# yhlleo/DWC-GAN

Hardware: AMD Instinct MI355X
Metric: CelebA 128x128 training images/sec (higher is better)
Workload: dtype f32; 1 GPU; BASELINE configs[1]: CelebA-shaped 128x128, per-GPU batch 16, fp32, full iteration (dis_update + gen_update + EMA + LR step), vgg_w=0, stride-1 3x3 / 5x5 and stride-2 4x4 layers (forward, data and weight gradient) as fp32-accurate TWO-plane f16 split products on the f16 MFMA (hi + lo 2^-11 per operand, per-tensor power-of-two scales, 3 products per multiply-add, matrix-core partial sums flushed to; image_size=128, per_gpu_batch=16, global_batch=16, parallelism=dp1

## Files before the change

### dwc-gan_amd/csrc/lstm.hip

```cpp
#include "dwc_common.h"

namespace {

__device__ __forceinline__ float sigmoidf_(float x) { return 1.f / (1.f + expf(-x)); }

template <int MT, int NB>
__device__ __forceinline__ void mfma_rows(const float* __restrict__ a_base, int row0, int a_rows, int a_pitch,
                                          const float* const (&b_rows)[NB], bool b_valid, int K, int q0, int q1,
                                          f32x4 (&acc)[NB][MT]) {
    constexpr int CH = (MT * NB <= 2) ? 8 : ((MT + NB <= 6) ? 5 : 3);
    const int lane = threadIdx.x & 63, r = lane & 15, j = lane >> 4;
    const float* a_row[MT];
    bool a_ok[MT];
#pragma unroll
    for (int m = 0; m < MT; ++m) {
        const int row = row0 + m * 16 + r;
        a_ok[m] = row < a_rows;
        a_row[m] = a_base + (size_t)min(row, a_rows - 1) * a_pitch;
    }
    for (int qc = q0; qc < q1; qc += CH) {
        f32x4 av[CH][MT], bv[CH][NB];
#pragma unroll
        for (int u = 0; u < CH; ++u) {
            const int kc = min(16 * (qc + u) + 4 * j, K - 4);
// ... 478 lines not shown
                if (!mine[k]) continue;
                const int p = threadIdx.x + 256 * k, b = b0 + (p >> 4), u = u0 + (p & 15);
                float* dg = dgates + (dTB + (size_t)t * B + b) * K + u;
                dg[0] = nan; dg[H] = nan; dg[2 * H] = nan; dg[3 * H] = nan;
            }
    }
}

template <typename K>
int lstm_resident_capacity(K kernel, unsigned dyn_lds, int variant) {
    static int cache[16][16];
    int dev = 0;
    if (hipGetDevice(&dev) != hipSuccess) return 0;
    int* slot = (dev >= 0 && dev < 16 && variant >= 0 && variant < 16) ? &cache[dev][variant] : nullptr;
    if (slot && *slot > 0) return *slot;
    int cus = 0, occ = 0;
    if (hipDeviceGetAttribute(&cus, hipDeviceAttributeMultiprocessorCount, dev) != hipSuccess) return 0;
    if (hipOccupancyMaxActiveBlocksPerMultiprocessor(&occ, kernel, 256, dyn_lds) != hipSuccess) return 0;
    const int cap = cus * occ;
    if (slot) *slot = cap;
    return cap;
}

}

extern "C" {

int dwc_lstm_fwd(const float* xproj, const float* w_hh, const int* lens, float* out, float* c, float* gates, int T, int B, int H,
                 int dirs, void* stream) {
    if (T <= 0 || B <= 0 || H <= 0 || (H & 3) || dirs < 1 || dirs > 2) return DWC_EINVAL;
    const int mt = min(4, (B + 15) / 16);
    const dim3 grid((H + 15) / 16, dirs, (B + 16 * mt - 1) / (16 * mt));
    hipStream_t st = (hipStream_t)stream;
    for (int s = 0; s < T; ++s) {
        switch (mt) {
            case 1: hipLaunchKernelGGL(lstm_step_fwd<1>, grid, dim3(256), 0, st, xproj, w_hh, lens, out, c, gates, T, B, H, s); break;
            case 2: hipLaunchKernelGGL(lstm_step_fwd<2>, grid, dim3(256), 0, st, xproj, w_hh, lens, out, c, gates, T, B, H, s); break;
            case 3: hipLaunchKernelGGL(lstm_step_fwd<3>, grid, dim3(256), 0, st, xproj, w_hh, lens, out, c, gates, T, B, H, s); break;
            default: hipLaunchKernelGGL(lstm_step_fwd<4>, grid, dim3(256), 0, st, xproj, w_hh, lens, out, c, gates, T, B, H, s); break;
        }
    }
    DWC_LAUNCH_CHECK();
    return DWC_OK;
}

size_t dwc_lstm_seq_ws_bytes(int B, int dirs) { return ((size_t)(16 + dirs * ((B + 63) / 16 + 1)) * sizeof(unsigned) + 64 + 15) / 16 * 16; }

int dwc_lstm_seq_fwd(const float* xproj, const float* w_hh, const int* lens, float* out, float* c, float* gates, int T, int B, int H,
                     int dirs, void* ws, size_t ws_bytes, unsigned* status, int max_workgroups, void* stream) {
// ... 94 lines not shown
```

### dwc-gan_amd/hipdwc/_lib.py

```python
import ctypes
import os

_HERE = os.path.dirname(os.path.abspath(__file__))
LIB_PATH = os.environ.get("DWC_HIP_LIB") or os.path.join(os.path.dirname(_HERE), "lib", "libdwcgan_hip.so")

c_fp = ctypes.c_void_p
c_int = ctypes.c_int
c_sz = ctypes.c_size_t
c_f = ctypes.c_float
c_u = ctypes.c_uint


class AdvSpec(ctypes.Structure):
    _fields_ = [("target", c_f * 4), ("w_src", c_f * 4), ("w_cls", c_f * 4)]


SIGNATURES = {
    "dwc_version": (c_int, []),
    "dwc_x3_gemm_mode": (c_int, [c_int]),
    "dwc_weight_prepared_elems": (c_sz, [c_int] * 8),
    "dwc_weight_prepare_fwd": (c_int, [c_fp, c_fp, c_int, c_int, c_int, c_int, c_int, c_int, c_fp]),
    "dwc_weight_prepare_dgrad": (c_int, [c_fp, c_fp, c_int, c_int, c_int, c_int, c_int, c_int, c_int, c_fp]),
    "dwc_conv2d_fwd_ws_bytes": (c_sz, [c_int] * 9),
    "dwc_conv2d_fwd": (c_int, [c_fp, c_fp, c_fp, c_fp] + [c_int] * 10 + [c_fp, c_sz, c_fp]),
# ... 54 lines not shown
    "dwc_bf16_conv2d_fwd_ex": (c_int, [c_fp, c_fp, c_fp, c_fp] + [c_int] * 12 + [c_fp]),
    "dwc_bf16_conv2d_bwd_data_ws_bytes": (c_sz, [c_int] * 9),
    "dwc_bf16_conv2d_bwd_data": (c_int, [c_fp, c_fp, c_fp] + [c_int] * 9 + [c_fp, c_sz, c_fp]),
    "dwc_bf16_conv2d_bwd_data_fold": (c_int, [c_fp, c_fp, c_fp, c_fp] + [c_int] * 9 + [c_fp, c_sz, c_fp]),
    "dwc_bf16_reflect_pad_adjoint": (c_int, [c_fp, c_fp, c_int, c_int, c_int, c_int, c_int, c_fp]),
    "dwc_bf16_reflect_pad_adjoint_band": (c_int, [c_fp, c_fp, c_int, c_int, c_int, c_int, c_int, c_fp]),
    "dwc_bf16_conv2d_bwd_data_same_ws_bytes": (c_sz, [c_int] * 8),
    "dwc_bf16_conv2d_bwd_data_same": (c_int, [c_fp] * 4 + [c_int] * 8 + [c_fp, c_sz, c_fp]),
    "dwc_bf16_conv2d_bwd_data_ring": (c_int, [c_fp] * 4 + [c_int] * 8 + [c_fp, c_sz, c_fp]),
    "dwc_bf16_conv2d_same_halo_ok": (c_int, [c_int] * 6),
    "dwc_bf16_conv2d_same_halo": (c_int, [c_fp] * 4 + [c_int] * 8 + [c_fp]),
    "dwc_bf16_conv2d_same_halo_add": (c_int, [c_fp] * 5 + [c_int] * 8 + [c_fp]),
    "dwc_bf16_conv2d_bwd_data_same_fused_ok": (c_int, [c_int] * 6),
    "dwc_bf16_conv2d_bwd_data_same_fused": (c_int, [c_fp] * 4 + [c_int] * 6 + [c_fp]),
    "dwc_weight_refresh_multi": (c_int, [c_fp, c_fp, c_fp, c_int, c_int, c_u, c_fp]),
    "dwc_bf16_conv2d_fwd_zeropad": (c_int, [c_fp, c_fp, c_fp, c_fp] + [c_int] * 10 + [c_fp, c_sz, c_fp]),
    "dwc_bf16_conv2d_bwd_data_zeropad_ws_bytes": (c_sz, [c_int] * 8),
    "dwc_bf16_conv2d_bwd_data_zeropad": (c_int, [c_fp, c_fp, c_fp] + [c_int] * 8 + [c_fp, c_sz, c_fp]),
    "dwc_bf16_maxpool2_fwd": (c_int, [c_fp, c_fp, c_int, c_int, c_int, c_int, c_fp]),
    "dwc_bf16_maxpool2_bwd": (c_int, [c_fp, c_fp, c_fp, c_int, c_int, c_int, c_int, c_fp]),
    "dwc_lstm_seq_ws_bytes": (c_sz, [c_int, c_int]),
    "dwc_lstm_seq_fwd": (c_int, [c_fp] * 6 + [c_int] * 4 + [c_fp, c_sz, c_fp, c_int, c_fp]),
    "dwc_lstm_seq_bwd": (c_int, [c_fp] * 7 + [c_int] * 4 + [c_fp, c_sz, c_fp, c_int, c_fp]),
    "dwc_adv_tail_fwd": (c_int, [c_fp, c_fp, c_fp, c_fp, c_int, c_int, c_int, c_int, AdvSpec, c_fp]),
    "dwc_adv_tail_bwd": (c_int, [c_fp, c_fp, c_fp, c_fp, c_fp, c_fp, c_int, c_int, c_int, c_int, AdvSpec, c_fp]),
    "dwc_bf16_conv2d_s2_halo_ok": (c_int, [c_int] * 5),
    "dwc_bf16_conv2d_s2_halo": (c_int, [c_fp] * 4 + [c_int] * 6 + [c_fp]),
    "dwc_x3_conv2d_same_ok": (c_int, [c_int] * 6),
    "dwc_x3_weight_prepared_elems": (c_sz, [c_int] * 3),
    "dwc_x3_weight_prepare": (c_int, [c_fp, c_fp] + [c_int] * 5 + [c_fp]),
    "dwc_x3_conv2d_same": (c_int, [c_fp] * 4 + [c_int] * 9 + [c_fp]),
    "dwc_x3_conv2d_same_add": (c_int, [c_fp] * 5 + [c_int] * 9 + [c_fp]),
    "dwc_x3_conv2d_narrow_ok": (c_int, [c_int] * 8),
    "dwc_x3_conv2d_narrow_weight_elems": (c_sz, [c_int] * 2),
    "dwc_x3_conv2d_narrow": (c_int, [c_fp] * 4 + [c_int] * 12 + [c_fp]),
    "dwc_reflect_pad_adjoint_pitch": (c_int, [c_fp, c_fp] + [c_int] * 6 + [c_fp]),
    "dwc_x3_gather_split": (c_int, [c_fp, c_fp, c_fp, c_int, c_fp]),
    "dwc_x3_conv2d_stem_ok": (c_int, [c_int] * 7),
    "dwc_x3_conv2d_stem_weight_elems": (c_sz, []),
    "dwc_x3_conv2d_stem": (c_int, [c_fp] * 4 + [c_int] * 9 + [c_fp]),
    "dwc_x3_conv2d_stem_crop": (c_int, [c_fp] * 5 + [c_int] * 10 + [c_fp]),
    "dwc_x3_conv2d_stem_amax": (c_int, [c_fp] * 5 + [c_u] + [c_int] * 9 + [c_fp]),
    "dwc_reflect_pad_adjoint_band": (c_int, [c_fp, c_fp, c_int, c_int, c_int, c_int, c_int, c_fp]),
    "dwc_x3_conv2d_ksplit_ws_bytes": (c_sz, [c_int] * 7),
    "dwc_x3_conv2d_ksplit_ticket_words": (c_int, []),
    "dwc_x3_conv2d_same_add_ws": (c_int, [c_fp] * 5 + [c_int] * 9 + [c_fp, c_sz, c_fp, c_fp]),
# ... 50 lines not shown
    "dwc_bf16_upsample2x_bwd": (c_int, [c_fp, c_fp, c_int, c_int, c_int, c_int, c_fp]),
    "dwc_bf16_avgpool2_fwd": (c_int, [c_fp, c_fp, c_int, c_int, c_int, c_int, c_fp]),
    "dwc_bf16_avgpool2_bwd": (c_int, [c_fp, c_fp, c_int, c_int, c_int, c_int, c_fp]),
    "dwc_pack_nchw_to_nhwc8_bf16": (c_int, [c_fp, c_fp, c_int, c_int, c_int, c_int, c_fp]),
    "dwc_unpack_nhwc8_bf16_to_nchw": (c_int, [c_fp, c_fp, c_int, c_int, c_int, c_int, c_fp]),
    "dwc_bf16_blend_fwd": (c_int, [c_fp, c_fp, c_fp, c_int, c_fp]),
    "dwc_bf16_blend_bwd": (c_int, [c_fp, c_fp, c_fp, c_fp, c_int, c_fp]),
    "dwc_bf16_l1_mean_fwd": (c_int, [c_fp, c_fp, c_fp, c_sz, c_int, c_fp, c_sz, c_fp]),
    "dwc_bf16_l1_mean_bwd": (c_int, [c_fp, c_fp, c_fp, c_fp, c_fp, c_sz, c_int, c_fp]),
    "dwc_sn_layer_saved_floats": (c_sz, [c_int] * 3),
    "dwc_sn_power_blocks": (c_int, [c_int, c_int, c_fp, c_fp]),
    "dwc_sn_power_iteration": (c_int, [c_fp, c_int, c_int, c_int, c_fp, c_int, c_fp]),
    "dwc_sn_epilogue_bwd_ws_bytes": (c_sz, [c_int] * 4),
    "dwc_sn_epilogue_fwd": (c_int, [c_fp] * 4 + [c_int] * 4 + [c_fp, c_u, c_fp]),
    "dwc_bf16_sn_epilogue_fwd": (c_int, [c_fp] * 4 + [c_int] * 4 + [c_fp]),
    "dwc_sn_epilogue_bwd": (c_int, [c_fp] * 7 + [c_int] * 4 + [c_fp, c_sz, c_fp, c_u, c_fp]),
    "dwc_bf16_sn_epilogue_bwd": (c_int, [c_fp] * 7 + [c_int] * 4 + [c_fp, c_sz, c_fp]),
    "dwc_sn_weight_grad": (c_int, [c_fp, c_int, c_fp, c_int, c_fp, c_fp, c_fp] + [c_int] * 4 + [c_fp]),
    "dwc_grad_penalty_fwd": (c_int, [c_fp] * 4 + [c_int] * 5 + [c_fp]),
    "dwc_grad_penalty_scale": (c_int, [c_fp] * 4 + [c_int] * 4 + [c_fp]),
    "dwc_src_head_seed": (c_int, [c_fp] * 3 + [c_int] * 3 + [c_fp]),
}

ABI_VERSION = 9
EINVAL = -1
_ERRORS = {-1: "DWC_EINVAL (unsupported shape/argument)", -2: "DWC_EWORKSPACE (scratch too small)",
           -3: "DWC_ELAUNCH (kernel launch failed)"}

_lib = None


class HipKernelError(RuntimeError):
    pass


def load():
    global _lib
    if _lib is not None:
        return _lib
    if not os.path.exists(LIB_PATH):
        raise ImportError(
            "libdwcgan_hip.so not found at %s — build it with `make -C dwc-gan_amd/csrc` "
            "(or python -c 'import __graft_entry__ as g; g.build()'). There is no CPU fallback." % LIB_PATH)
    import torch
    lib = ctypes.CDLL(LIB_PATH)
    for name, (res, args) in SIGNATURES.items():
        fn = getattr(lib, name)
# ... 14 lines not shown
```

### dwc-gan_amd/hipdwc/ops.py

```python
import os
import weakref

import numpy as np
import torch

from . import _lib

ACT = {"none": 0, None: 0, "relu": 1, "lrelu": 2, "tanh": 3, "sigmoid": 4, "heads": 5, "heads8": 6}

PRECISION = "fp32"
BF16 = torch.bfloat16

_REMOVED_SWITCHES = ("DWC_WINOGRAD", "DWC_TXT_STREAM", "DWC_NORM_FUSED_FINAL", "DWC_GEMM_TILE", "DWC_STRIP_BM", "DWC_X3_DUO", "DWC_X3_BN",
                     "DWC_X3_BN32", "DWC_X3_WIDE", "DWC_X3_STAGGER", "DWC_HALO_STAGGER", "DWC_X3_WDUO", "DWC_HALO16", "DWC_HALO_DUO",
                     "DWC_HALO_BN128", "DWC_BF16_TILE", "DWC_BF16_STAGES3", "DWC_NARROW_ROWS16")
_set = [k for k in _REMOVED_SWITCHES if k in os.environ]
if _set:
    import warnings
    warnings.warn("hipdwc: %s no longer select%s anything (removed in round 5, DESIGN.md 10.3) and %s ignored" % (
        ", ".join(_set), "s" if len(_set) == 1 else "", "is" if len(_set) == 1 else "are"), stacklevel=2)
del _set


def set_precision(name):
# ... 450 lines not shown
    _lib.check(lib.dwc_weight_refresh_multi(table[0].data_ptr(), table[1].data_ptr(), table[2].data_ptr(), table[3], table[4],
                                            _REFRESH_EPOCH, _stream()), "weight_refresh_multi")
    for p, ent, key, val, stamp in todo:
        ent[key] = (stamp, val[1], val[2])
    REFRESH_STATS["launches"] += 1
    REFRESH_STATS["layouts"] += len(todo)
    return len(todo)


X3 = int(os.environ.get("DWC_X3", "2"))
HALO = int(os.environ.get("DWC_BF16_HALO", "1"))
WGRAD_HALO = int(os.environ.get("DWC_BF16_WGRAD_HALO", "1"))
STEM = int(os.environ.get("DWC_BF16_STEM", "1"))
NARROW = int(os.environ.get("DWC_BF16_NARROW", "1"))
NARROW_X3 = int(os.environ.get("DWC_X3_NARROW", "1"))
SMALLK_X3 = int(os.environ.get("DWC_X3_SMALLK", "1"))
LSTM_SEQ = int(os.environ.get("DWC_LSTM_SEQ", "1"))
DGRAD_FOLD = int(os.environ.get("DWC_DGRAD_FOLD", "1"))
X3_S2 = int(os.environ.get("DWC_X3_S2", "1"))
S2HALO = int(os.environ.get("DWC_BF16_S2_HALO", "1"))
S2DGRAD = int(os.environ.get("DWC_S2_DGRAD_HALO", "1"))
X3_WGRAD_HALO3 = int(os.environ.get("DWC_X3_WGRAD_HALO3", "1"))
PINNED_STAGE = int(os.environ.get("DWC_PINNED_STAGE", "1"))
ZERO_GRAD_BY_FLAG = int(os.environ.get("DWC_ZERO_GRAD_FLAG", "1"))
RING_FUSED = int(os.environ.get("DWC_RING_FUSED", "1"))
PENALTY_HIP = int(os.environ.get("DWC_PENALTY_HIP", "0"))
S2DGRAD_MIN_WGS = 192


X3_PLANES = int(os.environ.get("DWC_X3_PLANES", "2"))
AMAX_SLOTS = 1 << 16
_AMAX = {}


def amax_slot(dev):
    key = dev.index if dev.index is not None else torch.cuda.current_device()
    pool = _AMAX.get(key)
    if pool is None:
        pool = [torch.zeros(AMAX_SLOTS, dtype=torch.int64, device=dev), 0]
        _AMAX[key] = pool
    i = pool[1]
    pool[1] = i + 1
    return pool[0].data_ptr() + 8 * (i % AMAX_SLOTS), i // AMAX_SLOTS + 1


def amax_live(t, c=False):
# ... 972 lines not shown
            ws = workspace(lib.dwc_lstm_seq_ws_bytes(B, 2), dev)
            rc = lib.dwc_lstm_seq_bwd(_p(d_out), _p(d_c), w_hh_t.data_ptr(), lens.data_ptr(), c.data_ptr(), gates.data_ptr(),
                                      dgates.data_ptr(), T, B, H, 2, ws.data_ptr(), ws.numel(), _lstm_status(dev)[0].data_ptr(),
                                      LSTM_SEQ_MAX_WORKGROUPS, _stream())
            if rc not in (0, _lib.EINVAL):
                _lib.check(rc, "lstm_seq_bwd")
        if rc != 0:
            _lib.check(lib.dwc_lstm_bwd(_p(d_out), _p(d_c), w_hh_t.data_ptr(), lens.data_ptr(), c.data_ptr(), gates.data_ptr(),
                                        dgates.data_ptr(), carry.data_ptr(), T, B, H, 2, _stream()), "lstm_bwd")
        dG = dgates.view(2, T * B, 4 * H)
        dGt = dG.transpose(1, 2)
        hip = ctx.hip_gemm
        dw_ih = None
        if ctx.needs_input_grad[2]:
            if hip:
                dw_ih = torch.empty((2, 4 * H, I), dtype=torch.float32, device=dev)
                for d in range(2):
                    _gemm_tn(dG[d], X, out=dw_ih[d])
            else:
                dw_ih = torch.matmul(dGt, X)
        db = dG.sum(1) if (ctx.needs_input_grad[4] or ctx.needs_input_grad[5]) else None
        dw_hh = None
        if ctx.needs_input_grad[3]:
            hprev = torch.zeros((2, T, B, H), dtype=torch.float32, device=dev)
            hprev[0, 1:] = out[0, :-1]
            hprev[1, :-1] = out[1, 1:]
            hp = hprev.view(2, T * B, H)
            if hip:
                dw_hh = torch.empty((2, 4 * H, H), dtype=torch.float32, device=dev)
                for d in range(2):
                    _gemm_tn(dG[d], hp[d], out=dw_hh[d])
            else:
                dw_hh = torch.bmm(dGt, hp)
        dx = None
        if ctx.needs_input_grad[0]:
            if hip:
                dx = (_gemm_nn(dG[0], w_ih[0], ctx.owners[0]) + _gemm_nn(dG[1], w_ih[1], ctx.owners[1])).view(T, B, I)
            else:
                dx = torch.bmm(dG, w_ih).sum(0).view(T, B, I)
        return dx, None, dw_ih, dw_hh, db, db, None


def lstm_bidir(x, lens, w_ih, w_hh, b_ih, b_hh, owners=None):
    return _LSTMBidir.apply(x.contiguous(), lens, w_ih, w_hh, b_ih, b_hh, owners)


class _InstNorm(torch.autograd.Function):
    @staticmethod
    def forward(ctx, x, gamma, beta, residual, relu, eps, token=None):
        _require_device(x)
        ctx.token = token if residual is not None else None
        lib = _lib.load()
        x = cl(x)
        B, C, H, W = x.shape
        dev = x.device
        if gamma is not None:
            gamma, beta = gamma.float().contiguous(), beta.float().contiguous()
        if residual is not None:
            residual = cl(residual.to(x.dtype))
        y = empty_cl(B, C, H, W, dev, x.dtype)
        mean = torch.empty(B * C, dtype=torch.float32, device=dev)
        rstd = torch.empty(B * C, dtype=torch.float32, device=dev)
        ws = workspace(lib.dwc_instnorm_ws_bytes(B, H * W, C), dev)
        ya, yep = out_amax(y)
        if ya is not None:
            _lib.check(lib.dwc_instnorm_fwd_amax(x.data_ptr(), _p(gamma), _p(beta), _p(residual), y.data_ptr(), mean.data_ptr(),
                                                 rstd.data_ptr(), B, H * W, C, eps, int(relu), ws.data_ptr(), ws.numel(),
# ... 360 lines not shown
```

### dwc-gan_amd/networks/networks_v2.py

```python
import numpy as np
import torch
from torch import nn

from hipdwc import host, ops
from .networks import ContentEncoder, MLP, Conv2dBlock, ResBlocks, AdaptiveInstanceNorm2d, Decoder


class HeadList(list):
    flat = None

    @classmethod
    def of(cls, flat, k):
        out = cls(flat.reshape(flat.shape[0], k, -1).unbind(1))
        out.flat = flat
        return out

    def rows(self, a, b):
        return HeadList.of(self.flat[a:b], len(self))


def flat_heads(heads):
    if torch.is_tensor(heads):
        return heads
    flat = getattr(heads, "flat", None)
# ... 81 lines not shown
            self.embed_tokens.weight.requires_grad = False
        self.lstm = nn.LSTM(input_size=embed_dim + self.style_dim, hidden_size=hidden_size, num_layers=num_layers,
                            dropout=dropout_out if num_layers > 1 else 0.0, bidirectional=bidirectional)
        feat = hidden_size * num_layers * (4 if bidirectional else 2)
        self.fcs, self.fcvars = nn.ModuleList(), nn.ModuleList()
        for _ in range(num_class):
            self.fcs.append(nn.Linear(feat, c_dim))
            self.fcvars.append(nn.Linear(feat, c_dim))

    def forward(self, style_ord, src_tokens, src_lengths):
        noise = host.noise()
        tokens = src_tokens.transpose(1, 0)
        seq_len, bsz = tokens.shape
        lens_host = src_lengths.detach().to("cpu")
        lens_sorted, order_host = torch.sort(lens_host, descending=True)
        if tokens.is_cuda and ops.PINNED_STAGE:
            stage = torch.empty(4, bsz, dtype=torch.int64).pin_memory()
            stage[0], stage[1], stage[2], stage[3] = order_host, torch.sort(order_host)[1], lens_sorted, lens_sorted - 1
            on_dev = stage.to(tokens.device, non_blocking=True)
            order, unsort, lens_dev, last = on_dev[0], on_dev[1], on_dev[2].to(torch.int32), on_dev[3]
        else:
            order, unsort = order_host.to(tokens.device), torch.sort(order_host)[1].to(tokens.device)
            lens_dev, last = lens_sorted.to(torch.int32).to(tokens.device), (lens_sorted - 1).to(tokens.device)
        emb = self.embed_tokens(tokens.index_select(1, order))
        emb = noise.dropout(emb, self.dropout_in, self.training)
        sty = _Permute.apply(style_ord, 0, order, unsort)
        lens_list = lens_sorted.tolist()
        t_max = int(lens_list[0])
        data = torch.cat([emb, sty.expand(seq_len, -1, -1)], -1)[:t_max]
        cols = torch.arange(bsz, device=tokens.device)
        suffixes = ("", "_reverse") if self.bidirectional else ("",)
        if not self.bidirectional:
            raise NotImplementedError("the HIP text encoder is bidirectional (the reference's only configuration)")
        hs, cs = [], []
        for l in range(self.num_layers):
            par = {n: ops.cat_params([getattr(self.lstm, "%s_l%d%s" % (n, l, suf)) for suf in suffixes], stack=True)
                   for n in ("weight_ih", "weight_hh", "bias_ih", "bias_hh")}
            out, cell = ops.lstm_bidir(data, lens_dev, par["weight_ih"], par["weight_hh"], par["bias_ih"], par["bias_hh"],
                                       owners=tuple(getattr(self.lstm, "weight_ih_l%d%s" % (l, suf)) for suf in suffixes))
            hs += [out[0][last, cols], out[1][0]]
            cs += [cell[0][last, cols], cell[1][0]]
            data = torch.cat([out[0], out[1]], -1)
            if l + 1 < self.num_layers and self.training and self.dropout_out > 0:
                if getattr(noise, "align_stream", False):
                    mask = noise.dropout_mask((int(sum(lens_list)), data.shape[2]), self.dropout_out, data.device)
                    data = data * mask.index_select(0, _packed_index(lens_list, t_max, bsz, data.device)).view(t_max, bsz, -1)
                else:
                    data = noise.dropout(data, self.dropout_out, True)
        h_n, c_n = torch.stack(hs), torch.stack(cs)
        if self.training and self.dropout_out > 0 and noise.align_stream:
            noise.dropout(data, self.dropout_out, True)
        h_n = h_n.view(self.num_layers, 2, bsz, -1).transpose(1, 2).reshape(self.num_layers, bsz, -1)
        c_n = c_n.view(self.num_layers, 2, bsz, -1).transpose(1, 2).reshape(self.num_layers, bsz, -1)
        h_n, c_n = _Permute.apply(h_n, 1, unsort, order), _Permute.apply(c_n, 1, unsort, order)
        feat = torch.cat([h_n, c_n], dim=1).view(bsz, -1)
        w = ops.cat_params([m.weight for m in self.fcs] + [m.weight for m in self.fcvars])
        b = ops.cat_params([m.bias for m in self.fcs] + [m.bias for m in self.fcvars])
        if feat.is_cuda and ops.LSTM_GEMM and ops.gemm_ok(feat.shape[1], w.shape[0]):
            out = ops.linear_any(feat, w, b, owner=tuple(m.weight for m in self.fcs) + tuple(m.weight for m in self.fcvars))
        else:
            out = torch.nn.functional.linear(feat, w, b)
        k, c = self.num_class, self.style_dim // self.num_class
        return HeadList.of(out[:, :k * c], k), HeadList.of(out[:, k * c:2 * k * c], k)


class AdaINGen_v2(nn.Module):

    def __init__(self, input_dim, vocab, params, pretrained_embed=None):
        super().__init__()
        p = params
        style_dim = p["c_dim"] * p["num_cls"]
        self.enc_style = StyleEncoder(p["style_downsample"], input_dim, p["dim"], norm="none", activ=p["activ"],
                                      pad_type=p["pad_type"], c_dim=p["c_dim"], num_class=p["num_cls"],
                                      use_map=p["use_map"])
        self.enc_content = ContentEncoder(p["content_downsample"], p["n_res"], input_dim, p["dim"], "in", p["activ"],
                                          pad_type=p["pad_type"])
        self.dec = Decoder(p["content_downsample"], p["n_res"], self.enc_content.output_dim, input_dim,
                           res_norm="adain", activ=p["activ"], pad_type=p["pad_type"],
# ... 50 lines not shown
```

### include/dwcgan_hip.h

```cpp
#ifndef DWCGAN_HIP_H
#define DWCGAN_HIP_H

#include <stddef.h>
#include <stdint.h>

#ifdef __cplusplus
extern "C" {
#endif

#define DWC_OK 0
#define DWC_EINVAL (-1)
#define DWC_EWORKSPACE (-2)
#define DWC_ELAUNCH (-3)

#define DWC_ACT_NONE 0
#define DWC_ACT_RELU 1
#define DWC_ACT_LRELU 2
#define DWC_ACT_TANH 3
#define DWC_ACT_SIGMOID 4
#define DWC_ACT_HEADS 5
#define DWC_ACT_HEADS8 6

#define DWC_ABI_VERSION 9
int dwc_version(void);
int dwc_x3_gemm_mode(int mode);

size_t dwc_weight_prepared_elems(int Cout, int Cin, int KH, int KW, int stride, int cout_pad, int cin_pad,
                                 int for_dgrad);
int dwc_weight_prepare_fwd(const float* w_oihw, float* w_prepared, int Cout, int Cin, int KH, int KW,
                           int cout_pad, int cin_pad, void* stream);
int dwc_weight_prepare_dgrad(const float* w_oihw, float* w_prepared, int Cout, int Cin, int KH, int KW,
                             int stride, int cout_pad, int cin_pad, void* stream);

size_t dwc_conv2d_fwd_ws_bytes(int B, int H, int W, int Cin, int Cout, int KH, int KW, int stride, int pad);
int dwc_conv2d_fwd(const float* x, const float* w_prepared, const float* bias, float* y,
                   int B, int H, int W, int Cin, int Cout, int KH, int KW, int stride, int pad,
                   int act, void* ws, size_t ws_bytes, void* stream);
size_t dwc_conv2d_bwd_data_ws_bytes(int B, int H, int W, int Cin, int Cout, int KH, int KW, int stride, int pad);
int dwc_conv2d_bwd_data(const float* dy, const float* w_dgrad, float* dxp,
                        int B, int H, int W, int Cin, int Cout, int KH, int KW, int stride, int pad,
                        void* ws, size_t ws_bytes, void* stream);
int dwc_reflect_pad_adjoint(const float* dxp, float* dx, int B, int H, int W, int C, int pad,
                            void* stream);
int dwc_conv2d_bwd_data_fold(const float* dy, const float* w_dgrad, float* dxp, float* dx, int B, int H, int W, int Cin, int Cout, int KH,
                             int KW, int stride, int pad, void* ws, size_t ws_bytes, void* stream);
size_t dwc_conv2d_bwd_data_same_ws_bytes(int B, int H, int W, int Cin, int Cout, int KH, int KW, int pad);
// ... 69 lines not shown
                  void* stream);

int dwc_gmm_kl_sp_fwd(const float* mu, const float* lv, const float* centre, int centre_stride, int B, int K, int D, float sigma,
                      float* out_scalar, void* stream);
int dwc_gmm_kl_sp_bwd(const float* mu, const float* lv, const float* centre, int centre_stride, int B, int K, int D, float sigma,
                      const float* dout_scalar, float* dmu, float* dlv, void* stream);

size_t dwc_l1_ws_bytes(size_t n);
int dwc_l1_mean_fwd(const float* a, const float* b, float* out_scalar, size_t n, int skip4, void* ws,
                    size_t ws_bytes, void* stream);
int dwc_l1_mean_bwd(const float* a, const float* b, const float* dout_scalar, float* da, float* db,
                    size_t n, int skip4, void* stream);

int dwc_lstm_fwd(const float* xproj, const float* w_hh, const int* lens, float* out, float* c, float* gates,
                 int T, int B, int H, int dirs, void* stream);
size_t dwc_lstm_seq_ws_bytes(int B, int dirs);
int dwc_lstm_seq_fwd(const float* xproj, const float* w_hh, const int* lens, float* out, float* c, float* gates, int T, int B, int H,
                     int dirs, void* ws, size_t ws_bytes, unsigned* status, int max_workgroups, void* stream);
int dwc_lstm_seq_bwd(const float* d_out, const float* d_c, const float* w_hh_t, const int* lens, const float* c, const float* gates,
                     float* dgates, int T, int B, int H, int dirs, void* ws, size_t ws_bytes, unsigned* status, int max_workgroups,
                     void* stream);
int dwc_lstm_bwd(const float* d_out, const float* d_c, const float* w_hh_t, const int* lens, const float* c,
                 const float* gates, float* dgates, float* dc_carry, int T, int B, int H, int dirs, void* stream);

int dwc_adam_step(float* p, const float* g, float* m, float* v, size_t n, float lr, float beta1,
                  float beta2, float eps, float weight_decay, int step, void* stream);
int dwc_ema_lerp(const float* p, float* ema, size_t n, float beta, void* stream);

#define DWC_OPT_CHUNK 8192
typedef struct {
    float* p;
    const float* g;
    float* m;
    float* v;
    unsigned long long n;
    float step_size;
    float bc2_sqrt;
} dwc_adam_tensor;
typedef struct {
    const float* p;
    float* ema;
    unsigned long long n;
} dwc_ema_tensor;
int dwc_adam_multi(const dwc_adam_tensor* tensors_dev, const int* chunk_tensor_dev,
                   const unsigned* chunk_start_dev, int n_chunks, double beta1, double beta2, double eps,
                   double weight_decay, void* stream);
// ... 235 lines not shown
```

Before: 398.3 images/s.

## Fuse text-encoder input assembly and final-state gather into HIP kernels

Adds HIP kernels that build the LSTM input in one pass: embedding lookup, token reordering, dropout mask and style concatenation. A second kernel gathers the final hidden and cell states and unsorts them, with matching backward kernels. The recurrent weight gradient now uses offset views of the outputs instead of materialising a zero-padded shifted copy. All of this replaces many small torch ops (index_select, cat, stack, permute) with fewer launches, at the cost of new custom autograd paths with fallbacks.

After: 401.1 images/s, median of 6. Within noise of the previous version (+0.7%).

```diff
diff --git a/dwc-gan_amd/csrc/lstm.hip b/dwc-gan_amd/csrc/lstm.hip
--- a/dwc-gan_amd/csrc/lstm.hip
+++ b/dwc-gan_amd/csrc/lstm.hip
@@ -524,9 +524,177 @@
     return cap;
 }
 
+
+constexpr int TXT_MAX_LAYERS = DWC_TXT_MAX_LAYERS;
+struct TxtStates { const float* out[TXT_MAX_LAYERS]; const float* c[TXT_MAX_LAYERS]; };
+struct TxtStateGrads { float* d_out[TXT_MAX_LAYERS]; float* d_c[TXT_MAX_LAYERS]; const float* addend[TXT_MAX_LAYERS]; };
+
+__global__ __launch_bounds__(256) void txt_input_fwd(const float* __restrict__ table, const long long* __restrict__ tokens,
+                                                     const long long* __restrict__ order, const float* __restrict__ mask,
+                                                     const float* __restrict__ style, float* __restrict__ data,
+                                                     long long* __restrict__ tok_t, int seq_len, int t_max, int B, int E, int S, int V) {
+    const int W = E + S;
+    const size_t n = (size_t)t_max * B * W, stride = (size_t)gridDim.x * 256;
+    const size_t i0 = (size_t)blockIdx.x * 256 + threadIdx.x;
+    for (size_t i = i0; i < n; i += stride) {
+        const int k = (int)(i % W);
+        const size_t row = i / W;
+        const int j = (int)(row % B), t = (int)(row / B);
+        const long long src = order[j];
+        float v = __builtin_nanf("");
+        if (src >= 0 && src < B) {
+            if (k < E) {
+                const long long tok = tokens[(size_t)src * seq_len + t];
+                if (tok >= 0 && tok < V) {
+                    v = table[(size_t)tok * E + k];
+                    if (mask) v = __fmul_rn(v, mask[row * E + k]);
+                }
+            } else {
+                v = style[(size_t)src * S + (k - E)];
+            }
+        }
+        data[i] = v;
+    }
+    if (tok_t) {
+        const size_t m = (size_t)seq_len * B;
+        for (size_t i = i0; i < m; i += stride) tok_t[i] = tokens[(i % B) * seq_len + i / B];
+    }
+}
+
+__global__ __launch_bounds__(256) void txt_input_bwd(const float* __restrict__ d_data, const long long* __restrict__ unsort,
+                                                     const float* __restrict__ mask, float* __restrict__ d_style,
+                                                     float* __restrict__ d_rows, int seq_len, int t_max, int B, int E, int S) {
+    const int W = E + S;
+    const size_t n_rows = d_rows ? (size_t)seq_len * B * E : 0, n_sty = d_style ? (size_t)B * S : 0;
+    const size_t stride = (size_t)gridDim.x * 256;
+    for (size_t i = (size_t)blockIdx.x * 256 + threadIdx.x; i < n_rows + n_sty; i += stride) {
+        if (i < n_rows) {
+            const int k = (int)(i % E);
+            const size_t row = i / E;
+            const int b = (int)(row % B), t = (int)(row / B);
+            const long long j = unsort[b];
+            float v = 0.f;
+            if (j < 0 || j >= B) {
+                v = __builtin_nanf("");
+            } else if (t < t_max) {
+                const size_t r = (size_t)t * B + j;
+                v = d_data[r * W + k];
+                if (mask) v = __fmul_rn(v, mask[r * E + k]);
+            }
+            d_rows[i] = v;
+        } else {
+            const size_t q = i - n_rows;
+            const int s = (int)(q % S), b = (int)(q / S);
+            const long long j = unsort[b];
+            float acc = 0.f;
+            if (j < 0 || j >= B) {
+                acc = __builtin_nanf("");
+            } else {
+                for (int t = 0; t < t_max; ++t) acc += d_data[((size_t)t * B + j) * W + E + s];
+            }
+            d_style[q] = acc;
+        }
+    }
+}
+
+__global__ __launch_bounds__(256) void txt_final_fwd(TxtStates p, const long long* __restrict__ last, const long long* __restrict__ unsort,
+                                                     float* __restrict__ feat, int L, int T, int B, int H) {
+    const size_t n = (size_t)L * 2 * B * 2 * H, stride = (size_t)gridDim.x * 256;
+    for (size_t i = (size_t)blockIdx.x * 256 + threadIdx.x; i < n; i += stride) {
+        const int k = (int)(i % (2 * H));
+        const int r = (int)((i / (2 * H)) % (2 * B)), l = (int)(i / ((size_t)4 * H * B));
+        const int d = k / H, h = k - d * H, b = r < B ? r : r - B;
+        const float* src = r < B ? p.out[l] : p.c[l];
+        const long long j = unsort[b];
+        float v = __builtin_nanf("");
+        if (j >= 0 && j < B) {
+            const long long t = d == 0 ? last[j] : 0;
+            if (t >= 0 && t < T) v = src[(((size_t)d * T + t) * B + j) * H + h];
+        }
+        feat[i] = v;
+    }
+}
+
+__global__ __launch_bounds__(256) void txt_final_bwd(TxtStateGrads p, const float* __restrict__ d_feat, const long long* __restrict__ last,
+                                                     const long long* __restrict__ order, int L, int T, int B, int H) {
+    const size_t per = (size_t)2 * T * B * H, n = (size_t)L * 2 * per, stride = (size_t)gridDim.x * 256;
+    for (size_t i = (size_t)blockIdx.x * 256 + threadIdx.x; i < n; i += stride) {
+        const size_t e = i % per;
+        const int which = (int)((i / per) & 1), l = (int)(i / (2 * per));
+        const int h = (int)(e % H), j = (int)((e / H) % B), t = (int)((e / ((size_t)H * B)) % T), d = (int)(e / ((size_t)H * B * T));
+        float v = 0.f;
+        if (d == 0 ? (long long)t == last[j] : t == 0) {
+            const long long b = order[j];
+            v = (b >= 0 && b < B) ? d_feat[(((size_t)l * 2 + which) * B + b) * 2 * H + d * H + h] : __builtin_nanf("");
+        }
+        if (which == 0) {
+            if (p.addend[l]) v += p.addend[l][((size_t)t * B + j) * 2 * H + d * H + h];
+            p.d_out[l][e] = v;
+        } else {
+            p.d_c[l][e] = v;
+        }
+    }
+}
+
+inline unsigned txt_blocks(size_t n) { return (unsigned)min((n + 255) / 256, (size_t)4096); }
+
 }
 
 extern "C" {
+
+int dwc_txt_input_fwd(const float* table, const long long* tokens, const long long* order, const float* mask, const float* style,
+                      float* data, long long* tok_t, int seq_len, int t_max, int B, int E, int S, int V, void* stream) {
+    if (!table || !tokens || !order || !style || !data) return DWC_EINVAL;
+    if (seq_len <= 0 || t_max <= 0 || t_max > seq_len || B <= 0 || E <= 0 || S <= 0 || V <= 0) return DWC_EINVAL;
+    if ((size_t)seq_len * B * (E + S) >= 0x80000000ull || (size_t)V * E >= 0x80000000ull) return DWC_EINVAL;
+    const size_t n = max((size_t)t_max * B * (E + S), tok_t ? (size_t)seq_len * B : (size_t)0);
+    hipLaunchKernelGGL(txt_input_fwd, dim3(txt_blocks(n)), dim3(256), 0, (hipStream_t)stream, table, tokens, order, mask, style, data,
+                       tok_t, seq_len, t_max, B, E, S, V);
+    DWC_LAUNCH_CHECK();
+    return DWC_OK;
+}
+
+int dwc_txt_input_bwd(const float* d_data, const long long* unsort, const float* mask, float* d_style, float* d_rows, int seq_len,
+                      int t_max, int B, int E, int S, void* stream) {
+    if (!d_data || !unsort || (!d_style && !d_rows)) return DWC_EINVAL;
+    if (seq_len <= 0 || t_max <= 0 || t_max > seq_len || B <= 0 || E <= 0 || S <= 0) return DWC_EINVAL;
+    if ((size_t)seq_len * B * (E + S) >= 0x80000000ull) return DWC_EINVAL;
+    const size_t n = (d_rows ? (size_t)seq_len * B * E : 0) + (d_style ? (size_t)B * S : 0);
+    hipLaunchKernelGGL(txt_input_bwd, dim3(txt_blocks(n)), dim3(256), 0, (hipStream_t)stream, d_data, unsort, mask, d_style, d_rows,
+                       seq_len, t_max, B, E, S);
+    DWC_LAUNCH_CHECK();
+    return DWC_OK;
+}
+
+int dwc_txt_final_fwd(const float* const* outs, const float* const* cs, const long long* last, const long long* unsort, float* feat,
+                      int L, int T, int B, int H, void* stream) {
+    if (!outs || !cs || !last || !unsort || !feat || L <= 0 || L > TXT_MAX_LAYERS || T <= 0 || B <= 0 || H <= 0) return DWC_EINVAL;
+    if ((size_t)2 * T * B * H >= 0x80000000ull || (size_t)L * 4 * B * H >= 0x80000000ull) return DWC_EINVAL;
+    TxtStates p = {};
+    for (int l = 0; l < L; ++l) {
+        if (!outs[l] || !cs[l]) return DWC_EINVAL;
+        p.out[l] = outs[l], p.c[l] = cs[l];
+    }
+    hipLaunchKernelGGL(txt_final_fwd, dim3(txt_blocks((size_t)L * 4 * B * H)), dim3(256), 0, (hipStream_t)stream, p, last, unsort, feat,
+                       L, T, B, H);
+    DWC_LAUNCH_CHECK();
+    return DWC_OK;
+}
+
+int dwc_txt_final_bwd(const float* d_feat, const long long* last, const long long* order, float* const* d_outs, float* const* d_cs,
+                      const float* const* addends, int L, int T, int B, int H, void* stream) {
+    if (!d_feat || !last || !order || !d_outs || !d_cs || L <= 0 || L > TXT_MAX_LAYERS || T <= 0 || B <= 0 || H <= 0) return DWC_EINVAL;
+    if ((size_t)2 * T * B * H >= 0x80000000ull || (size_t)L * 4 * B * H >= 0x80000000ull) return DWC_EINVAL;
+    TxtStateGrads p = {};
+    for (int l = 0; l < L; ++l) {
+        if (!d_outs[l] || !d_cs[l]) return DWC_EINVAL;
+        p.d_out[l] = d_outs[l], p.d_c[l] = d_cs[l], p.addend[l] = addends ? addends[l] : nullptr;
+    }
+    hipLaunchKernelGGL(txt_final_bwd, dim3(txt_blocks((size_t)L * 4 * T * B * H)), dim3(256), 0, (hipStream_t)stream, p, d_feat, last,
+                       order, L, T, B, H);
+    DWC_LAUNCH_CHECK();
+    return DWC_OK;
+}
 
 int dwc_lstm_fwd(const float* xproj, const float* w_hh, const int* lens, float* out, float* c, float* gates, int T, int B, int H,
                  int dirs, void* stream) {
diff --git a/dwc-gan_amd/hipdwc/_lib.py b/dwc-gan_amd/hipdwc/_lib.py
--- a/dwc-gan_amd/hipdwc/_lib.py
+++ b/dwc-gan_amd/hipdwc/_lib.py
@@ -100,6 +100,10 @@
     "dwc_lstm_seq_ws_bytes": (c_sz, [c_int, c_int]),
     "dwc_lstm_seq_fwd": (c_int, [c_fp] * 6 + [c_int] * 4 + [c_fp, c_sz, c_fp, c_int, c_fp]),
     "dwc_lstm_seq_bwd": (c_int, [c_fp] * 7 + [c_int] * 4 + [c_fp, c_sz, c_fp, c_int, c_fp]),
+    "dwc_txt_input_fwd": (c_int, [c_fp] * 7 + [c_int] * 6 + [c_fp]),
+    "dwc_txt_input_bwd": (c_int, [c_fp] * 5 + [c_int] * 5 + [c_fp]),
+    "dwc_txt_final_fwd": (c_int, [c_fp] * 5 + [c_int] * 4 + [c_fp]),
+    "dwc_txt_final_bwd": (c_int, [c_fp] * 6 + [c_int] * 4 + [c_fp]),
     "dwc_adv_tail_fwd": (c_int, [c_fp, c_fp, c_fp, c_fp, c_int, c_int, c_int, c_int, AdvSpec, c_fp]),
     "dwc_adv_tail_bwd": (c_int, [c_fp, c_fp, c_fp, c_fp, c_fp, c_fp, c_int, c_int, c_int, c_int, AdvSpec, c_fp]),
     "dwc_bf16_conv2d_s2_halo_ok": (c_int, [c_int] * 5),
@@ -196,7 +200,7 @@
     "dwc_src_head_seed": (c_int, [c_fp] * 3 + [c_int] * 3 + [c_fp]),
 }
 
-ABI_VERSION = 9
+ABI_VERSION = 10
 EINVAL = -1
 _ERRORS = {-1: "DWC_EINVAL (unsupported shape/argument)", -2: "DWC_EWORKSPACE (scratch too small)",
            -3: "DWC_ELAUNCH (kernel launch failed)"}
diff --git a/dwc-gan_amd/hipdwc/ops.py b/dwc-gan_amd/hipdwc/ops.py
--- a/dwc-gan_amd/hipdwc/ops.py
+++ b/dwc-gan_amd/hipdwc/ops.py
@@ -1,3 +1,4 @@
+import ctypes
 import os
 import weakref
 
@@ -496,6 +497,7 @@
 S2DGRAD = int(os.environ.get("DWC_S2_DGRAD_HALO", "1"))
 X3_WGRAD_HALO3 = int(os.environ.get("DWC_X3_WGRAD_HALO3", "1"))
 PINNED_STAGE = int(os.environ.get("DWC_PINNED_STAGE", "1"))
+TXT_FUSED = int(os.environ.get("DWC_TXT_FUSED", "1"))
 ZERO_GRAD_BY_FLAG = int(os.environ.get("DWC_ZERO_GRAD_FLAG", "1"))
 RING_FUSED = int(os.environ.get("DWC_RING_FUSED", "1"))
 PENALTY_HIP = int(os.environ.get("DWC_PENALTY_HIP", "0"))
@@ -1514,16 +1516,22 @@
         db = dG.sum(1) if (ctx.needs_input_grad[4] or ctx.needs_input_grad[5]) else None
         dw_hh = None
         if ctx.needs_input_grad[3]:
-            hprev = torch.zeros((2, T, B, H), dtype=torch.float32, device=dev)
-            hprev[0, 1:] = out[0, :-1]
-            hprev[1, :-1] = out[1, 1:]
-            hp = hprev.view(2, T * B, H)
-            if hip:
+            if hip and TXT_FUSED and T > 1:
                 dw_hh = torch.empty((2, 4 * H, H), dtype=torch.float32, device=dev)
-                for d in range(2):
-                    _gemm_tn(dG[d], hp[d], out=dw_hh[d])
+                o = out.view(2, T * B, H)
+                _gemm_tn(dG[0, B:], o[0, :(T - 1) * B], out=dw_hh[0])
+                _gemm_tn(dG[1, :(T - 1) * B], o[1, B:], out=dw_hh[1])
             else:
-                dw_hh = torch.bmm(dGt, hp)
+                hprev = torch.zeros((2, T, B, H), dtype=torch.float32, device=dev)
+                hprev[0, 1:] = out[0, :-1]
+                hprev[1, :-1] = out[1, 1:]
+                hp = hprev.view(2, T * B, H)
+                if hip:
+                    dw_hh = torch.empty((2, 4 * H, H), dtype=torch.float32, device=dev)
+                    for d in range(2):
+                        _gemm_tn(dG[d], hp[d], out=dw_hh[d])
+                else:
+                    dw_hh = torch.bmm(dGt, hp)
         dx = None
         if ctx.needs_input_grad[0]:
             if hip:
@@ -1535,6 +1543,105 @@
 
 def lstm_bidir(x, lens, w_ih, w_hh, b_ih, b_hh, owners=None):
     return _LSTMBidir.apply(x.contiguous(), lens, w_ih, w_hh, b_ih, b_hh, owners)
+
+
+class _TxtUnsupported(Exception):
+    """A dwc_txt_* entry point returned DWC_EINVAL: the caller assembles the tensor with torch ops."""
+
+
+def _txt_call(rc, what):
+    if rc == _lib.EINVAL:
+        raise _TxtUnsupported(what)
+    _lib.check(rc, what)
+
+
+def _ptr_array(tensors):
+    return (ctypes.c_void_p * len(tensors))(*[_p(t) for t in tensors])
+
+
+class _TxtInput(torch.autograd.Function):
+
+    @staticmethod
+    def forward(ctx, table, style, tokens, order, unsort, mask, t_max, padding_idx):
+        B, seq_len = tokens.shape
+        (V, E), S = table.shape, style.shape[1]
+        data = torch.empty((t_max, B, E + S), dtype=torch.float32, device=table.device)
+        tok_t = torch.empty((seq_len, B), dtype=torch.int64, device=table.device) if ctx.needs_input_grad[0] else None
+        _txt_call(_lib.load().dwc_txt_input_fwd(table.data_ptr(), tokens.data_ptr(), order.data_ptr(), _p(mask), style.data_ptr(),
+                                                data.data_ptr(), _p(tok_t), seq_len, t_max, B, E, S, V, _stream()), "txt_input_fwd")
+        ctx.save_for_backward(unsort, mask, tok_t)
+        ctx.dims = (seq_len, t_max, B, E, S, V, -1 if padding_idx is None else int(padding_idx))
+        return data
+
+    @staticmethod
+    def backward(ctx, d_data):
+        unsort, mask, tok_t = ctx.saved_tensors
+        seq_len, t_max, B, E, S, V, pad = ctx.dims
+        d_data = d_data.contiguous()
+        dev = d_data.device
+        d_rows = torch.empty((seq_len, B, E), dtype=torch.float32, device=dev) if ctx.needs_input_grad[0] else None
+        d_style = torch.empty((B, S), dtype=torch.float32, device=dev) if ctx.needs_input_grad[1] else None
+        if d_rows is not None or d_style is not None:
+            _lib.check(_lib.load().dwc_txt_input_bwd(d_data.data_ptr(), unsort.data_ptr(), _p(mask), _p(d_style), _p(d_rows), seq_len,
+                                                     t_max, B, E, S, _stream()), "txt_input_bwd")
+        d_table = None if d_rows is None else torch.ops.aten.embedding_dense_backward(d_rows, tok_t, V, pad, False)
+        return d_table, d_style, None, None, None, None, None, None
+
+
+def _txt_plain(*tensors):
+    return all(t is None or (t.is_cuda and t.is_contiguous()) for t in tensors)
+
+
+def txt_input(table, padding_idx, tokens, order, unsort, mask, style, t_max):
+    if not (TXT_FUSED and _txt_plain(table, tokens, order, unsort, mask, style) and tokens.dtype == torch.int64
+            and order.dtype == torch.int64 and unsort.dtype == torch.int64 and table.dtype == torch.float32
+            and style.dtype == torch.float32 and (mask is None or mask.dtype == torch.float32)):
+        return None
+    try:
+        return _TxtInput.apply(table, style, tokens, order, unsort, mask, int(t_max), padding_idx)
+    except _TxtUnsupported:
+        return None
+
+
+class _TxtFinal(torch.autograd.Function):
+
+    @staticmethod
+    def forward(ctx, last, unsort, order, *states):
+        L = len(states) // 2
+        _, T, B, H = states[0].shape
+        feat = torch.empty((B, 4 * L * H), dtype=torch.float32, device=states[0].device)
+        _txt_call(_lib.load().dwc_txt_final_fwd(_ptr_array(states[0::2]), _ptr_array(states[1::2]), last.data_ptr(), unsort.data_ptr(),
+                                                feat.data_ptr(), L, T, B, H, _stream()), "txt_final_fwd")
+        ctx.save_for_backward(last, order)
+        ctx.dims = (L, T, B, H)
+        return feat
+
+    @staticmethod
+    def backward(ctx, d_feat):
+        last, order = ctx.saved_tensors
+        L, T, B, H = ctx.dims
+        grads = txt_final_bwd(d_feat.contiguous(), last, order, L, T, H)
+        return (None, None, None) + tuple(g for pair in zip(*grads) for g in pair)
+
+
+def txt_final_bwd(d_feat, last, order, L, T, H, addends=None):
+    B = d_feat.shape[0]
+    d_outs = [torch.empty((2, T, B, H), dtype=torch.float32, device=d_feat.device) for _ in range(L)]
+    d_cs = [torch.empty((2, T, B, H), dtype=torch.float32, device=d_feat.device) for _ in range(L)]
+    _lib.check(_lib.load().dwc_txt_final_bwd(d_feat.data_ptr(), last.data_ptr(), order.data_ptr(), _ptr_array(d_outs), _ptr_array(d_cs),
+                                             None if addends is None else _ptr_array(addends), L, T, B, H, _stream()), "txt_final_bwd")
+    return d_outs, d_cs
+
+
+def txt_final(last, unsort, order, outs, cells):
+    states = [t for pair in zip(outs, cells) for t in pair]
+    if not (TXT_FUSED and _txt_plain(last, unsort, order, *states) and all(t.dtype == torch.float32 for t in states)
+            and all(t.dtype == torch.int64 for t in (last, unsort, order))):
+        return None
+    try:
+        return _TxtFinal.apply(last, unsort, order, *states)
+    except _TxtUnsupported:
+        return None
 
 
 class _InstNorm(torch.autograd.Function):
diff --git a/dwc-gan_amd/networks/networks_v2.py b/dwc-gan_amd/networks/networks_v2.py
--- a/dwc-gan_amd/networks/networks_v2.py
+++ b/dwc-gan_amd/networks/networks_v2.py
@@ -127,38 +127,52 @@
         else:
             order, unsort = order_host.to(tokens.device), torch.sort(order_host)[1].to(tokens.device)
             lens_dev, last = lens_sorted.to(torch.int32).to(tokens.device), (lens_sorted - 1).to(tokens.device)
-        emb = self.embed_tokens(tokens.index_select(1, order))
-        emb = noise.dropout(emb, self.dropout_in, self.training)
-        sty = _Permute.apply(style_ord, 0, order, unsort)
         lens_list = lens_sorted.tolist()
         t_max = int(lens_list[0])
-        data = torch.cat([emb, sty.expand(seq_len, -1, -1)], -1)[:t_max]
-        cols = torch.arange(bsz, device=tokens.device)
+        fused = tokens.is_cuda and ops.TXT_FUSED
+        data = mask = None
+        if fused:
+            if self.training and self.dropout_in > 0:
+                mask = noise.dropout_mask((seq_len, bsz, self.embed_dim), self.dropout_in, tokens.device)
+            data = ops.txt_input(self.embed_tokens.weight, self.embed_tokens.padding_idx, src_tokens.contiguous(), order, unsort, mask,
+                                 style_ord, t_max)
+        if data is None:
+            emb = self.embed_tokens(tokens.index_select(1, order))
+            emb = emb * mask if mask is not None else noise.dropout(emb, self.dropout_in, self.training)
+            sty = _Permute.apply(style_ord, 0, order, unsort)
+            data = torch.cat([emb, sty.expand(seq_len, -1, -1)], -1)[:t_max]
         suffixes = ("", "_reverse") if self.bidirectional else ("",)
         if not self.bidirectional:
             raise NotImplementedError("the HIP text encoder is bidirectional (the reference's only configuration)")
-        hs, cs = [], []
+        outs, cells = [], []
         for l in range(self.num_layers):
             par = {n: ops.cat_params([getattr(self.lstm, "%s_l%d%s" % (n, l, suf)) for suf in suffixes], stack=True)
                    for n in ("weight_ih", "weight_hh", "bias_ih", "bias_hh")}
             out, cell = ops.lstm_bidir(data, lens_dev, par["weight_ih"], par["weight_hh"], par["bias_ih"], par["bias_hh"],
                                        owners=tuple(getattr(self.lstm, "weight_ih_l%d%s" % (l, suf)) for suf in suffixes))
-            hs += [out[0][last, cols], out[1][0]]
-            cs += [cell[0][last, cols], cell[1][0]]
-            data = torch.cat([out[0], out[1]], -1)
+            outs.append(out)
+            cells.append(cell)
+            if fused and l + 1 == self.num_layers and not noise.align_stream:
+                break
+            data = out.permute(1, 2, 0, 3).reshape(t_max, bsz, -1) if fused else torch.cat([out[0], out[1]], -1)
             if l + 1 < self.num_layers and self.training and self.dropout_out > 0:
                 if getattr(noise, "align_stream", False):
-                    mask = noise.dropout_mask((int(sum(lens_list)), data.shape[2]), self.dropout_out, data.device)
-                    data = data * mask.index_select(0, _packed_index(lens_list, t_max, bsz, data.device)).view(t_max, bsz, -1)
+                    pmask = noise.dropout_mask((int(sum(lens_list)), data.shape[2]), self.dropout_out, data.device)
+                    data = data * pmask.index_select(0, _packed_index(lens_list, t_max, bsz, data.device)).view(t_max, bsz, -1)
                 else:
                     data = noise.dropout(data, self.dropout_out, True)
-        h_n, c_n = torch.stack(hs), torch.stack(cs)
         if self.training and self.dropout_out > 0 and noise.align_stream:
             noise.dropout(data, self.dropout_out, True)
-        h_n = h_n.view(self.num_layers, 2, bsz, -1).transpose(1, 2).reshape(self.num_layers, bsz, -1)
-        c_n = c_n.view(self.num_layers, 2, bsz, -1).transpose(1, 2).reshape(self.num_layers, bsz, -1)
-        h_n, c_n = _Permute.apply(h_n, 1, unsort, order), _Permute.apply(c_n, 1, unsort, order)
-        feat = torch.cat([h_n, c_n], dim=1).view(bsz, -1)
+        feat = ops.txt_final(last, unsort, order, outs, cells) if fused else None
+        if feat is None:
+            cols = torch.arange(bsz, device=tokens.device)
+            hs = [h for out in outs for h in (out[0][last, cols], out[1][0])]
+            cs = [c for cell in cells for c in (cell[0][last, cols], cell[1][0])]
+            h_n, c_n = torch.stack(hs), torch.stack(cs)
+            h_n = h_n.view(self.num_layers, 2, bsz, -1).transpose(1, 2).reshape(self.num_layers, bsz, -1)
+            c_n = c_n.view(self.num_layers, 2, bsz, -1).transpose(1, 2).reshape(self.num_layers, bsz, -1)
+            h_n, c_n = _Permute.apply(h_n, 1, unsort, order), _Permute.apply(c_n, 1, unsort, order)
+            feat = torch.cat([h_n, c_n], dim=1).view(bsz, -1)
         w = ops.cat_params([m.weight for m in self.fcs] + [m.weight for m in self.fcvars])
         b = ops.cat_params([m.bias for m in self.fcs] + [m.bias for m in self.fcvars])
         if feat.is_cuda and ops.LSTM_GEMM and ops.gemm_ok(feat.shape[1], w.shape[0]):
diff --git a/include/dwcgan_hip.h b/include/dwcgan_hip.h
--- a/include/dwcgan_hip.h
+++ b/include/dwcgan_hip.h
@@ -21,7 +21,7 @@
 #define DWC_ACT_HEADS 5
 #define DWC_ACT_HEADS8 6
 
-#define DWC_ABI_VERSION 9
+#define DWC_ABI_VERSION 10
 int dwc_version(void);
 int dwc_x3_gemm_mode(int mode);
 
@@ -137,6 +137,16 @@
                      void* stream);
 int dwc_lstm_bwd(const float* d_out, const float* d_c, const float* w_hh_t, const int* lens, const float* c,
                  const float* gates, float* dgates, float* dc_carry, int T, int B, int H, int dirs, void* stream);
+
+#define DWC_TXT_MAX_LAYERS 8
+int dwc_txt_input_fwd(const float* table, const long long* tokens, const long long* order, const float* mask, const float* style,
+                      float* data, long long* tok_t, int seq_len, int t_max, int B, int E, int S, int V, void* stream);
+int dwc_txt_input_bwd(const float* d_data, const long long* unsort, const float* mask, float* d_style, float* d_rows, int seq_len,
+                      int t_max, int B, int E, int S, void* stream);
+int dwc_txt_final_fwd(const float* const* outs, const float* const* cs, const long long* last, const long long* unsort, float* feat,
+                      int L, int T, int B, int H, void* stream);
+int dwc_txt_final_bwd(const float* d_feat, const long long* last, const long long* order, float* const* d_outs, float* const* d_cs,
+                      const float* const* addends, int L, int T, int B, int H, void* stream);
 
 int dwc_adam_step(float* p, const float* g, float* m, float* v, size_t n, float lr, float beta1,
                   float beta2, float eps, float weight_decay, int step, void* stream);
```
